# idiap/juicer

Measured on AMD Instinct MI355X. Metric: frames/sec decoded, higher is better.
Workload: dtype f32

## Files before the change

juicer_amd/build.py:

```python
from __future__ import annotations

import os
import shutil
import subprocess
import sys

HERE = os.path.dirname(os.path.abspath(__file__))
ROOT = os.path.dirname(HERE)
CSRC = os.path.join(HERE, "csrc")
LIB = os.path.join(HERE, "libjuicer_amd.so")
BATCH_TEST = os.path.join(HERE, "jd_batch_test")
BATCH_SRC = os.path.join(CSRC, "jd_batch_test.cpp")
SOURCES = [os.path.join(CSRC, "jd_host.cpp"), os.path.join(CSRC, "jd_device.hip"), os.path.join(CSRC, "jd_multi.cpp"),
           os.path.join(CSRC, "jd_compose.hip"), os.path.join(CSRC, "jd_broker.cpp")]
HEADERS_EXTRA = [os.path.join(CSRC, f) for f in ("jd_search.h", "jd_prep.h", "jd_lazy.h", "jd_labelsets.h", "jd_gmm.h", "jd_gc.h", "jd_resident.h", "jd_slot.h", "jd_host_resident.h", "jd_host_scoring.h", "jd_plan.h", "jd_host_launch.h", "jd_host_stream.h")]
HEADERS = [os.path.join(CSRC, "jd_internal.h"), os.path.join(ROOT, "include", "juicer_amd.h"),
           os.path.join(ROOT, "include", "juicer_amd_decoder.hpp"), BATCH_SRC]
FLAGS = ["--offload-arch=gfx950", "-O3", "-std=c++17", "-ffp-contract=off", "-fPIC", "-shared",
         "-Wall", "-Wno-unused-function"]


def hipcc() -> str:
    exe = shutil.which("hipcc") or "/opt/rocm/bin/hipcc"
    if not os.path.exists(exe):
        raise RuntimeError("hipcc not found: juicer_amd needs ROCm to build its HIP extension")
    return exe


def needs_build() -> bool:
    if not os.path.exists(LIB) or not os.path.exists(BATCH_TEST):
        return True
    t = os.path.getmtime(LIB)
    return any(os.path.getmtime(p) > t for p in SOURCES + HEADERS + HEADERS_EXTRA + [__file__])


def build(force: bool = False, verbose: bool = False) -> str:
    if not force and not needs_build():
        return LIB
    cmd = [hipcc()] + FLAGS + os.environ.get("JD_EXTRA_FLAGS", "").split() + ["-I", os.path.join(ROOT, "include"), "-I", CSRC, "-o", LIB] + SOURCES
    if verbose:
        print(" ".join(cmd), file=sys.stderr)
    subprocess.check_call(cmd)
    cmd2 = ["g++", "-O2", "-std=c++17", "-Wall", "-pthread", "-I", os.path.join(ROOT, "include"), "-o", BATCH_TEST, BATCH_SRC,
            "-L", HERE, "-ljuicer_amd", "-Wl,-rpath,$ORIGIN", "-Wl,-rpath-link," + "/opt/rocm/lib"]
    if verbose:
        print(" ".join(cmd2), file=sys.stderr)
    subprocess.check_call(cmd2)
    return LIB


if __name__ == "__main__":
    print(build(force="--force" in sys.argv, verbose=True))
```

juicer_amd/csrc/jd_gmm.h:

```cpp
#pragma once

#define JD_EXP2F_TAB                                                                              \
    0x3ff0000000000000ULL, 0x3fefd9b0d3158574ULL, 0x3fefb5586cf9890fULL, 0x3fef9301d0125b51ULL,   \
    0x3fef72b83c7d517bULL, 0x3fef54873168b9aaULL, 0x3fef387a6e756238ULL, 0x3fef1e9df51fdee1ULL,   \
    0x3fef06fe0a31b715ULL, 0x3feef1a7373aa9cbULL, 0x3feedea64c123422ULL, 0x3feece086061892dULL,   \
    0x3feebfdad5362a27ULL, 0x3feeb42b569d4f82ULL, 0x3feeab07dd485429ULL, 0x3feea47eb03a5585ULL,   \
    0x3feea09e667f3bcdULL, 0x3fee9f75e8ec5f74ULL, 0x3feea11473eb0187ULL, 0x3feea589994cce13ULL,   \
    0x3feeace5422aa0dbULL, 0x3feeb737b0cdc5e5ULL, 0x3feec49182a3f090ULL, 0x3feed503b23e255dULL,   \
    0x3feee89f995ad3adULL, 0x3feeff76f2fb5e47ULL, 0x3fef199bdd85529cULL, 0x3fef3720dcef9069ULL,   \
    0x3fef5818dcfba487ULL, 0x3fef7c97337b9b5fULL, 0x3fefa4afa2a490daULL, 0x3fefd0765b6e4540ULL
__device__ __constant__ unsigned long long jd_exp2f_tab[32] = {JD_EXP2F_TAB};
static const unsigned long long jd_exp2f_tab_host[32] = {JD_EXP2F_TAB};

__host__ __device__ __forceinline__ float jd_expf_impl(float x, const unsigned long long *tab)
{
    const double InvLn2N = 0x1.71547652b82fep+0 * 32.0;
    const double SHIFT = 0x1.8p+52;
    const double C0 = 0x1.c6af84b912394p-5 / 32.0 / 32.0 / 32.0;
    const double C1 = 0x1.ebfce50fac4f3p-3 / 32.0 / 32.0;
    const double C2 = 0x1.62e42ff0c52d6p-1 / 32.0;
    double z = InvLn2N * (double)x;
    double kd = z + SHIFT;
    unsigned long long ki;
    memcpy(&ki, &kd, sizeof ki);
    kd -= SHIFT;
    double r = z - kd;
    unsigned long long t = tab[ki & 31];
    t += ki << 47;
    double s;
    memcpy(&s, &t, sizeof s);
    double p = C0 * r + C1;
    double r2 = r * r;
    double y = C2 * r + 1.0;
    y = p * r2 + y;
    y = y * s;
    return (float)y;
}
__device__ __forceinline__ float jd_expf(float x) { return jd_expf_impl(x, jd_exp2f_tab); }

#define JD_LOG_TAB                                                                                          \
    0x3ff734f0c3e0de9fULL, 0xbfd7cc7f79e69000ULL, 0x3ff713786a2ce91fULL, 0xbfd76feec20d0000ULL,   \
    0x3ff6f26008fab5a0ULL, 0xbfd713e31351e000ULL, 0x3ff6d1a61f138c7dULL, 0xbfd6b85b38287800ULL,   \
    0x3ff6b1490bc5b4d1ULL, 0xbfd65d5590807800ULL, 0x3ff69147332f0cbaULL, 0xbfd602d076180000ULL,   \
    0x3ff6719f18224223ULL, 0xbfd5a8ca86909000ULL, 0x3ff6524f99a51ed9ULL, 0xbfd54f4356035000ULL,   \
    0x3ff63356aa8f24c4ULL, 0xbfd4f637c36b4000ULL, 0x3ff614b36b9ddc14ULL, 0xbfd49da7fda85000ULL,   \
    0x3ff5f66452c65c4cULL, 0xbfd445923989a800ULL, 0x3ff5d867b5912c4fULL, 0xbfd3edf439b0b800ULL,   \
    0x3ff5babccb5b90deULL, 0xbfd396ce448f7000ULL, 0x3ff59d61f2d91a78ULL, 0xbfd3401e17bda000ULL,   \
    0x3ff5805612465687ULL, 0xbfd2e9e2ef468000ULL, 0x3ff56397cee76bd3ULL, 0xbfd2941b3830e000ULL,   \
    0x3ff54725e2a77f93ULL, 0xbfd23ec58cda8800ULL, 0x3ff52aff42064583ULL, 0xbfd1e9e129279000ULL,   \
    0x3ff50f22dbb2bddfULL, 0xbfd1956d2b48f800ULL, 0x3ff4f38f4734ded7ULL, 0xbfd141679ab9f800ULL,   \
    0x3ff4d843cfde2840ULL, 0xbfd0edd094ef9800ULL, 0x3ff4bd3ec078a3c8ULL, 0xbfd09aa518db1000ULL,   \
    0x3ff4a27fc3e0258aULL, 0xbfd047e65263b800ULL, 0x3ff4880524d48434ULL, 0xbfcfeb224586f000ULL,   \
    0x3ff46dce1b192d0bULL, 0xbfcf474a7517b000ULL, 0x3ff453d9d3391854ULL, 0xbfcea4443d103000ULL,   \
    0x3ff43a2744b4845aULL, 0xbfce020d44e9b000ULL, 0x3ff420b54115f8fbULL, 0xbfcd60a22977f000ULL,   \
    0x3ff40782da3ef4b1ULL, 0xbfccc00104959000ULL, 0x3ff3ee8f5d57fe8fULL, 0xbfcc202956891000ULL,   \
    0x3ff3d5d9a00b4ce9ULL, 0xbfcb81178d811000ULL, 0x3ff3bd60c010c12bULL, 0xbfcae2c9ccd3d000ULL,   \
    0x3ff3a5242b75dab8ULL, 0xbfca45402e129000ULL, 0x3ff38d22cd9fd002ULL, 0xbfc9a877681df000ULL,   \
    0x3ff3755bc5847a1cULL, 0xbfc90c6d69483000ULL, 0x3ff35dce49ad36e2ULL, 0xbfc87120a645c000ULL,   \
    0x3ff34679984dd440ULL, 0xbfc7d68fb4143000ULL, 0x3ff32f5cceffcb24ULL, 0xbfc73cb83c627000ULL,   \
    0x3ff3187775a10d49ULL, 0xbfc6a39a9b376000ULL, 0x3ff301c8373e3990ULL, 0xbfc60b3154b7a000ULL,   \
    0x3ff2eb4ebb95f841ULL, 0xbfc5737d76243000ULL, 0x3ff2d50a0219a9d1ULL, 0xbfc4dc7b8fc23000ULL,   \
    0x3ff2bef9a8b7fd2aULL, 0xbfc4462c51d20000ULL, 0x3ff2a91c7a0c1babULL, 0xbfc3b08abc830000ULL,   \
    0x3ff293726014b530ULL, 0xbfc31b996b490000ULL, 0x3ff27dfa5757a1f5ULL, 0xbfc2875490a44000ULL,   \
    0x3ff268b39b1d3bbfULL, 0xbfc1f3b9f879a000ULL, 0x3ff2539d838ff5bdULL, 0xbfc160c8252ca000ULL,   \
    0x3ff23eb7aac9083bULL, 0xbfc0ce7f57f72000ULL, 0x3ff22a012ba940b6ULL, 0xbfc03cdc49fea000ULL,   \
    0x3ff2157996cc4132ULL, 0xbfbf57bdbc4b8000ULL, 0x3ff201201dd2fc9bULL, 0xbfbe370896404000ULL,   \
    0x3ff1ecf4494d480bULL, 0xbfbd17983ef94000ULL, 0x3ff1d8f5528f6569ULL, 0xbfbbf9674ed8a000ULL,   \
    0x3ff1c52311577e7cULL, 0xbfbadc79202f6000ULL, 0x3ff1b17c74cb26e9ULL, 0xbfb9c0c3e7288000ULL,   \
    0x3ff19e010c2c1ab6ULL, 0xbfb8a646b372c000ULL, 0x3ff18ab07bb670bdULL, 0xbfb78d01b3ac0000ULL,   \
    0x3ff1778a25efbcb6ULL, 0xbfb674f145380000ULL, 0x3ff1648d354c31daULL, 0xbfb55e0e6d878000ULL,   \
    0x3ff151b990275fddULL, 0xbfb4485cdea1e000ULL, 0x3ff13f0ea432d24cULL, 0xbfb333d94d6aa000ULL,   \
    0x3ff12c8b7210f9daULL, 0xbfb22079f8c56000ULL, 0x3ff11a3028ecb531ULL, 0xbfb10e4698622000ULL,   \
    0x3ff107fbda8434afULL, 0xbfaffa6c6ad20000ULL, 0x3ff0f5ee0f4e6bb3ULL, 0xbfadda8d4a774000ULL,   \
    0x3ff0e4065d2a9fceULL, 0xbfabbcece4850000ULL, 0x3ff0d244632ca521ULL, 0xbfa9a1894012c000ULL,   \
    0x3ff0c0a77ce2981aULL, 0xbfa788583302c000ULL, 0x3ff0af2f83c636d1ULL, 0xbfa5715e67d68000ULL,   \
    0x3ff09ddb98a01339ULL, 0xbfa35c8a49658000ULL, 0x3ff08cabaf52e7dfULL, 0xbfa149e364154000ULL,   \
    0x3ff07b9f2f4e28fbULL, 0xbf9e72c082eb8000ULL, 0x3ff06ab58c358f19ULL, 0xbf9a55f152528000ULL,   \
    0x3ff059eea5ecf92cULL, 0xbf963d62cf818000ULL, 0x3ff04949cdd12c90ULL, 0xbf9228fb8caa0000ULL,   \
    0x3ff038c6c6f0ada9ULL, 0xbf8c317b20f90000ULL, 0x3ff02865137932a9ULL, 0xbf8419355daa0000ULL,   \
    0x3ff0182427ea7348ULL, 0xbf781203c2ec0000ULL, 0x3ff008040614b195ULL, 0xbf60040979240000ULL,   \
    0x3fefe01ff726fa1aULL, 0x3f6feff384900000ULL, 0x3fefa11cc261ea74ULL, 0x3f87dc41353d0000ULL,   \
    0x3fef6310b081992eULL, 0x3f93cea3c4c28000ULL, 0x3fef25f63ceeadcdULL, 0x3f9b9fc114890000ULL,   \
    0x3feee9c8039113e7ULL, 0x3fa1b0d8ce110000ULL, 0x3feeae8078cbb1abULL, 0x3fa58a5bd001c000ULL,   \
    0x3fee741aa29d0c9bULL, 0x3fa95c8340d88000ULL, 0x3fee3a91830a99b5ULL, 0x3fad276aef578000ULL,   \
    0x3fee01e009609a56ULL, 0x3fb07598e598c000ULL, 0x3fedca01e577bb98ULL, 0x3fb253f5e30d2000ULL,   \
    0x3fed92f20b7c9103ULL, 0x3fb42edd8b380000ULL, 0x3fed5cac66fb5cceULL, 0x3fb606598757c000ULL,   \
    0x3fed272caa5ede9dULL, 0x3fb7da76356a0000ULL, 0x3fecf26e3e6b2ccdULL, 0x3fb9ab434e1c6000ULL,   \
    0x3fecbe6da2a77902ULL, 0x3fbb78c7bb0d6000ULL, 0x3fec8b266d37086dULL, 0x3fbd431332e72000ULL,   \
    0x3fec5894bd5d5804ULL, 0x3fbf0a3171de6000ULL, 0x3fec26b533bb9f8cULL, 0x3fc067152b914000ULL,   \
    0x3febf583eeece73fULL, 0x3fc147858292b000ULL, 0x3febc4fd75db96c1ULL, 0x3fc2266ecdca3000ULL,   \
    0x3feb951e0c864a28ULL, 0x3fc303d7a6c55000ULL, 0x3feb65e2c5ef3e2cULL, 0x3fc3dfc33c331000ULL,   \
    0x3feb374867c9888bULL, 0x3fc4ba366b7a8000ULL, 0x3feb094b211d304aULL, 0x3fc5933928d1f000ULL,   \
    0x3feadbe885f2ef7eULL, 0x3fc66acd2418f000ULL, 0x3feaaf1d31603da2ULL, 0x3fc740f8ec669000ULL,   \
    0x3fea82e63fd358a7ULL, 0x3fc815c0f51af000ULL, 0x3fea5740ef09738bULL, 0x3fc8e92954f68000ULL,   \
    0x3fea2c2a90ab4b27ULL, 0x3fc9bb3602f84000ULL, 0x3fea01a01393f2d1ULL, 0x3fca8bed1c2c0000ULL,   \
    0x3fe9d79f24db3c1bULL, 0x3fcb5b515c01d000ULL, 0x3fe9ae2505c7b190ULL, 0x3fcc2967ccbcc000ULL,   \
    0x3fe9852ef297ce2fULL, 0x3fccf635d5486000ULL, 0x3fe95cbaeea44b75ULL, 0x3fcdc1bd3446c000ULL,   \
    0x3fe934c69de74838ULL, 0x3fce8c01b8cfe000ULL, 0x3fe90d4f2f6752e6ULL, 0x3fcf5509c0179000ULL,   \
    0x3fe8e6528effd79dULL, 0x3fd00e6c121fb800ULL, 0x3fe8bfce9fcc007cULL, 0x3fd071b80e93d000ULL,   \
    0x3fe899c0dabec30eULL, 0x3fd0d46b9e867000ULL, 0x3fe87427aa2317fbULL, 0x3fd13687334bd000ULL,   \
    0x3fe84f00acb39a08ULL, 0x3fd1980d67234800ULL, 0x3fe82a49e8653e55ULL, 0x3fd1f8ffe0cc8000ULL,   \
    0x3fe8060195f40260ULL, 0x3fd2595fd7636800ULL, 0x3fe7e22563e0a329ULL, 0x3fd2b9300914a800ULL,   \
    0x3fe7beb377dcb5adULL, 0x3fd3187210436000ULL, 0x3fe79baa679725c2ULL, 0x3fd377266dec1800ULL,   \
    0x3fe77907f2170657ULL, 0x3fd3d54ffbaf3000ULL, 0x3fe756cadbd6130cULL, 0x3fd432eee32fe000ULL
__device__ __constant__ unsigned long long jd_log_tab[256] = {JD_LOG_TAB};
static const unsigned long long jd_log_tab_host[256] = {JD_LOG_TAB};

__host__ __device__ __forceinline__ double jd_u2d(unsigned long long u) { double d; memcpy(&d, &u, sizeof d); return d; }
__host__ __device__ __forceinline__ unsigned long long jd_d2u(double d) { unsigned long long u; memcpy(&u, &d, sizeof u); return u; }

__host__ __device__ inline double jd_log_libm_impl(double x, const unsigned long long *tab)
{
    const unsigned long long ix = jd_d2u(x);
    if (ix - 0x3fee000000000000ULL < 0x3ff1090000000000ULL - 0x3fee000000000000ULL) {
        if (ix == 0x3ff0000000000000ULL) return 0.0;
        const double r = x - 1.0, r2 = r * r, r3 = r * r2;
        double p = __builtin_fma(r, -0x1.ffffffffffdcbp-3, 0x1.5555555555577p-2);
        p = __builtin_fma(r2, 0x1.999999995dd0cp-3, p);
        double q = __builtin_fma(r, 0x1.24924a344de30p-3, -0x1.55555556745a7p-3);
        q = __builtin_fma(r2, -0x1.fffffa4423d65p-4, q);
        double s = __builtin_fma(r, -0x1.999eb43b068ffp-4, 0x1.c7184282ad6cap-4);
        s = __builtin_fma(r2, 0x1.78182f7afd085p-4, s);
        s = __builtin_fma(r3, -0x1.5521375d145cdp-4, s);
        s = __builtin_fma(s, r3, q);
        s = __builtin_fma(s, r3, p);
        const double rhi = __builtin_fma(-r, 0x1p27, __builtin_fma(r, 0x1p27, r));
        const double rlo = r - rhi;
        const double rr = rhi * rhi;
        const double hi = __builtin_fma(rr, -0.5, r);
        double lo = __builtin_fma(rr, -0.5, r - hi);
        lo = __builtin_fma(rlo * -0.5, r + rhi, lo);
        return hi + __builtin_fma(s, r3, lo);
    }
    const unsigned long long tmp = ix - 0x3fe6000000000000ULL;
    const int i = (int)((tmp >> 45) & 127);
    const double kd = (double)((long long)tmp >> 52);
    const double z = jd_u2d(ix - (tmp & (0xfffULL << 52)));
    const double invc = jd_u2d(tab[2 * i]), logc = jd_u2d(tab[2 * i + 1]);
    const double r = __builtin_fma(z, invc, -1.0);
    const double w = __builtin_fma(kd, 0x1.62e42fefa3800p-1, logc);
    const double hi = w + r;
    const double lo = __builtin_fma(kd, 0x1.ef35793c76730p-45, (w - hi) + r);
    const double r2 = r * r;
    const double p = __builtin_fma(__builtin_fma(r, -0x1.55575e506c89fp-3, 0x1.999b324f10111p-3), r2,
                                   __builtin_fma(r, -0x1.fffffffeb4590p-3, 0x1.555555551305bp-2));
    return __builtin_fma(r * r2, p, __builtin_fma(r2, -0x1.0000000000001p-1, lo)) + hi;
}

struct JdLogTab { double invc, logc; };
static inline void jd_fill_logtab(JdLogTab *t)
{
    for (int k = 0; k <= 128; ++k) {
        const double c = 1.0 + k / 128.0;
        t[k].invc = (k == 0) ? 1.0 : 1.0 / c;
        t[k].logc = (k == 0) ? 0.0 : (double)(-logl((long double)t[k].invc));
    }
}
__host__ __device__ __forceinline__ double jd_log1pe_table(double e, const JdLogTab *tab)
{
    const JdLogTab t = tab[(int)(e * 128.0 + 0.5)];
    const double r = __builtin_fma(1.0 + e, t.invc, -1.0);
    double q = 1.0 / 7.0;
    q = __builtin_fma(q, r, -1.0 / 6.0);
    q = __builtin_fma(q, r, 1.0 / 5.0);
    q = __builtin_fma(q, r, -1.0 / 4.0);
    q = __builtin_fma(q, r, 1.0 / 3.0);
    q = __builtin_fma(q, r, -1.0 / 2.0);
    q = __builtin_fma(q, r, 1.0);
    return t.logc + q * r;
}

__host__ __device__ __forceinline__ bool jd_log_add_gate(float a, float c, const JdLogTab *tab, const unsigned long long *etab,
                                                         float &x, float &d, double &y, float &n)
{
    const bool s = a < c;
    x = s ? c : a;
    d = (s ? a : c) - x;
    const double e = (double)jd_expf_impl(fmaxf(d, -19.0f), etab);
    y = 1.0 + e;
    const unsigned long long m = jd_d2u(jd_log1pe_table(e, tab));
    n = (float)((double)x + jd_u2d(m - 2));
    return d >= -18.42 && n != (float)((double)x + jd_u2d(m + 2));
}
__host__ __device__ __forceinline__ float jd_log_add_settle(float x, float d, float n)
{
    return d < -18.42 ? x : (d != d ? d : n);
}
__host__ __device__ __forceinline__ float jd_log_add_impl(float a, float c, const JdLogTab *tab, const unsigned long long *etab,
                                                          const unsigned long long *ltab)
{
    float x, d, n;
    double y;
    if (jd_log_add_gate(a, c, tab, etab, x, d, y, n)) n = (float)((double)x + jd_log_libm_impl(y, ltab));
    return jd_log_add_settle(x, d, n);
}
__device__ __forceinline__ float jd_log_add(float a, float c, const JdLogTab *tab)
{
    return jd_log_add_impl(a, c, tab, jd_exp2f_tab, jd_log_tab);
}


template <int DT>
__global__ __launch_bounds__(256) void jd_gmm_kernel(const float *__restrict__ feats,
                                                     const int *__restrict__ row_src, int n_rows,
                                                     const float *__restrict__ par,
                                                     const float *__restrict__ det,
                                                     const int *__restrict__ n_mix, int G, int M, int D,
                                                     float *__restrict__ ll, int skip_unused,
                                                     const JdLogTab *__restrict__ logtab)
{
    constexpr int DP = (DT > 0) ? (DT | 1) : 0;
    extern __shared__ __align__(16) char smem[];
    const int dp = (DT > 0) ? DP : (D | 1);
    float *sx = (float *)smem;
    float *so = sx + GMM_ROWS * dp;
    const int tid = threadIdx.x, lane = tid & 63;
    const int wid = __builtin_amdgcn_readfirstlane(tid >> 6);
    const int Dn = (DT > 0) ? DT : D;
    const int n_rt = (n_rows + GMM_ROWS - 1) / GMM_ROWS, n_gt = (G + GMM_GT - 1) / GMM_GT;
    for (int tile = blockIdx.x; tile < n_rt * n_gt; tile += gridDim.x) {
    const int gt = tile / n_rt;
    const int r0 = ((tile + gt) % n_rt) * GMM_ROWS;
    const int g0 = gt * GMM_GT;
    if (skip_unused && row_src[r0] < 0) continue;
    __syncthreads();

    for (int e = tid; e < GMM_ROWS * Dn; e += 256) {
        int r = e / Dn, j = e - r * Dn;
        int src = (r0 + r < n_rows) ? row_src[r0 + r] : -1;
        sx[r * dp + j] = (src >= 0) ? feats[(size_t)src * Dn + j] : 0.0f;
    }
    __syncthreads();

    float x[(DT > 0) ? DT : 1];
    if (DT > 0) {
#pragma unroll
        for (int j = 0; j < DT; ++j) x[j] = sx[lane * dp + j];
    }

    constexpr int GPW = GMM_GT / 4;
    for (int gi = 0; gi < GPW; ++gi) {
        const int gl = wid * GPW + gi;
        const int g = g0 + gl;
        float acc = LZ;
        if (g < G) {
            const int nm = n_mix[g];
            const float *pg = par + (size_t)g * M * Dn * 2;
            const float *dg = det + (size_t)g * M;
            for (int m = 0; m < nm; ++m) {
                const float *pm = pg + (size_t)m * Dn * 2;
                float sum = 0.0f;
                if (DT > 0) {
#pragma unroll
                    for (int j = 0; j < DT; ++j) {
                        float xmu = x[j] - pm[2 * j];
                        sum += xmu * xmu * pm[2 * j + 1];
                    }
                } else {
                    for (int j = 0; j < Dn; ++j) {
                        float xmu = sx[lane * dp + j] - pm[2 * j];
                        sum += xmu * xmu * pm[2 * j + 1];
                    }
                }
                float comp = (float)(-0.5 * (double)sum + (double)dg[m]);
                acc = jd_log_add(acc, comp, logtab);
            }
        }
        so[lane * (GMM_GT + 1) + gl] = acc;
    }
    __syncthreads();
    for (int e = tid; e < GMM_ROWS * GMM_GT; e += 256) {
        int r = e / GMM_GT, c = e - r * GMM_GT;
        if (r0 + r < n_rows && g0 + c < G) ll[(size_t)(r0 + r) * G + g0 + c] = so[r * (GMM_GT + 1) + c];
    }
    }
}


#define GMM_ROWS2 128
typedef float jd_f2 __attribute__((ext_vector_type(2)));
__host__ __device__ __forceinline__ void jd_log_add2x2(float &a0, float &a1, float c0, float c1, const JdLogTab *tab,
                                                       const unsigned long long *etab)
{
    float x0, x1, d0, d1, n0, n1;
    double y0, y1;
    const bool o0 = jd_log_add_gate(a0, c0, tab, etab, x0, d0, y0, n0);
    const bool o1 = jd_log_add_gate(a1, c1, tab, etab, x1, d1, y1, n1);
    a0 = o0 ? __builtin_nanf("") : jd_log_add_settle(x0, d0, n0);
    a1 = o1 ? __builtin_nanf("") : jd_log_add_settle(x1, d1, n1);
}

__device__ __noinline__ float jd_gmm_cell39(const float *__restrict__ feats, const int *__restrict__ row_src, int n_rows, int r,
                                            const float *__restrict__ pg, const float *__restrict__ dg, int nm,
                                            const JdLogTab *tab, const unsigned long long *etab)
{
    const int src = (r < n_rows) ? row_src[r] : -1;
    float acc = LZ;
    for (int m = 0; m < nm; ++m) {
        const float *pm = pg + (size_t)m * 39 * 2;
        float sum = 0.0f;
        for (int j = 0; j < 39; ++j) {
            const float u = ((src >= 0) ? feats[(size_t)src * 39 + j] : 0.0f) - pm[2 * j];
            const float z = u * u * pm[2 * j + 1];
            sum = (j == 0) ? z : sum + z;
        }
        const float c = (float)(-0.5 * (double)sum + (double)dg[m]);
        acc = (m == 0) ? (c <= LZ ? LZ : c) : jd_log_add_impl(acc, c, tab, etab, jd_log_tab);
    }
    return acc;
}

template <int GT>
__global__ __launch_bounds__(256, 4) void jd_gmm_kernel39(const float *__restrict__ feats,
                                                       const int *__restrict__ row_src, int n_rows,
                                                       const float *__restrict__ par,
                                                       const float *__restrict__ det,
                                                       const int *__restrict__ n_mix, int G, int M,
                                                       float *__restrict__ ll, int skip_unused,
                                                       const JdLogTab *__restrict__ logtab,
                                                       const int *__restrict__ rt_base, int n_rt_list)
{
    constexpr int DT = 39, DP = 39;
    extern __shared__ __align__(16) char smem[];
    JdLogTab *stab = (JdLogTab *)smem;
    unsigned long long *setab = (unsigned long long *)(smem + 130 * sizeof(JdLogTab));
    float *sx = (float *)(smem + 130 * sizeof(JdLogTab) + 32 * sizeof(unsigned long long));
    float *so = sx;
    const int tid = threadIdx.x, lane = tid & 63;
    const int wid = __builtin_amdgcn_readfirstlane(tid >> 6);
    for (int i = tid; i < 129; i += 256) stab[i] = logtab[i];
    if (tid < 32) setab[tid] = jd_exp2f_tab[tid];
    const int n_rt = rt_base ? n_rt_list : (n_rows + GMM_ROWS2 - 1) / GMM_ROWS2, n_gt = (G + GT - 1) / GT;
    for (int tile = blockIdx.x; tile < n_rt * n_gt; tile += gridDim.x) {
        const int gt = tile / n_rt;
        const int r0 = rt_base ? rt_base[(tile + gt) % n_rt] : ((tile + gt) % n_rt) * GMM_ROWS2;
        const int g0 = gt * GT;
        if (skip_unused && row_src[r0] < 0) continue;
        __syncthreads();
        for (int e = tid; e < GMM_ROWS2 * DT; e += 256) {
            const int r = e / DT, j = e - r * DT;
            const int src = (r0 + r < n_rows) ? row_src[r0 + r] : -1;
            sx[r * DP + j] = (src >= 0) ? feats[(size_t)src * DT + j] : 0.0f;
        }
        __syncthreads();
        jd_f2 x[DT];
#pragma unroll
        for (int j = 0; j < DT; ++j) { x[j].x = sx[lane * DP + j]; x[j].y = sx[(lane + 64) * DP + j]; }
        __syncthreads();
        constexpr int GPW = GT / 4;
        static_assert(GPW <= 16, "one bit per (state, frame) of a lane in open_cells");
        unsigned open_cells = 0;
        for (int gi = 0; gi < GPW; ++gi) {
            const int gl = wid * GPW + gi;
            const int g = g0 + gl;
            float acc0 = LZ, acc1 = LZ;
            if (g < G) {
                const int nm = n_mix[g];
                const float *pg = par + (size_t)g * M * DT * 2;
                const float *dg = det + (size_t)g * M;
                for (int m = 0; m < nm; ++m) {
                    const float *pm = pg + (size_t)m * DT * 2;
                    jd_f2 sum = {0.0f, 0.0f};
#pragma unroll
                    for (int j = 0; j < DT; j += 3) {
                        const jd_f2 mu0 = {pm[2 * j], pm[2 * j]}, iv0 = {pm[2 * j + 1], pm[2 * j + 1]};
                        const jd_f2 mu1 = {pm[2 * j + 2], pm[2 * j + 2]}, iv1 = {pm[2 * j + 3], pm[2 * j + 3]};
                        const jd_f2 mu2 = {pm[2 * j + 4], pm[2 * j + 4]}, iv2 = {pm[2 * j + 5], pm[2 * j + 5]};
                        const jd_f2 u0 = x[j] - mu0, u1 = x[j + 1] - mu1, u2 = x[j + 2] - mu2;
                        const jd_f2 w0 = u0 * u0, w1 = u1 * u1, w2 = u2 * u2;
                        const jd_f2 z0 = w0 * iv0, z1 = w1 * iv1, z2 = w2 * iv2;
                        if (j == 0) sum = z0; else sum += z0;
                        sum += z1; sum += z2;
                    }
                    const double dm = (double)dg[m];
                    const float c0 = (float)(-0.5 * (double)sum.x + dm), c1 = (float)(-0.5 * (double)sum.y + dm);
                    if (m == 0) { acc0 = c0 <= LZ ? LZ : c0; acc1 = c1 <= LZ ? LZ : c1; }
                    else jd_log_add2x2(acc0, acc1, c0, c1, stab, setab);
                }
            }
            so[lane * (GT + 1) + gl] = acc0;
            so[(lane + 64) * (GT + 1) + gl] = acc1;
            open_cells |= (acc0 != acc0 ? 1u << gi : 0u) | (acc1 != acc1 ? 1u << (16 + gi) : 0u);
        }
        for (unsigned o = open_cells; o; o &= o - 1) {
            const int b = __builtin_ctz(o), gl = wid * GPW + (b & 15), fr = b >> 4;
            const int g = g0 + gl;
            so[(lane + 64 * fr) * (GT + 1) + gl] = jd_gmm_cell39(feats, row_src, n_rows, r0 + lane + 64 * fr, par + (size_t)g * M * DT * 2,
                                                                det + (size_t)g * M, n_mix[g], stab, setab);
        }
        __syncthreads();
        for (int e = tid; e < GMM_ROWS2 * GT; e += 256) {
            const int r = e / GT, c = e - r * GT;
            if (r0 + r < n_rows && g0 + c < G) ll[(size_t)(r0 + r) * G + g0 + c] = so[r * (GT + 1) + c];
        }
    }
}


__device__ __forceinline__ float jd_log_add_fast(float a, float c)
{
    const float x = fmaxf(a, c), y = fminf(a, c);
    const float d = y - x;
    const float e = __builtin_amdgcn_exp2f(d * 1.44269504088896340736f);
    const float l = __builtin_amdgcn_logf(1.0f + e) * 0.69314718055994530942f;
    return d < -18.42f ? x : x + l;
}

template <int GT>
__global__ __launch_bounds__(256, 4) void jd_gmm_fast39(const float *__restrict__ feats, const int *__restrict__ row_src, int n_rows,
                                                      const float *__restrict__ par_fast, const float *__restrict__ det,
                                                      const int *__restrict__ n_mix, int G, int M, float *__restrict__ ll, int skip_unused,
                                                      const int *__restrict__ rt_base, int n_rt_list)
{
    constexpr int DT = 39, DP = 39;
    extern __shared__ __align__(16) char smem[];
    float *sx = (float *)smem;
    float *so = sx;
    const int tid = threadIdx.x, lane = tid & 63;
    const int wid = __builtin_amdgcn_readfirstlane(tid >> 6);
    const int n_rt = rt_base ? n_rt_list : (n_rows + GMM_ROWS2 - 1) / GMM_ROWS2, n_gt = (G + GT - 1) / GT;
    for (int tile = blockIdx.x; tile < n_rt * n_gt; tile += gridDim.x) {
        const int gt = tile / n_rt;
        const int r0 = rt_base ? rt_base[(tile + gt) % n_rt] : ((tile + gt) % n_rt) * GMM_ROWS2;
        const int g0 = gt * GT;
        if (skip_unused && row_src[r0] < 0) continue;
        __syncthreads();
        for (int e = tid; e < GMM_ROWS2 * DT; e += 256) {
            const int r = e / DT, j = e - r * DT;
            const int src = (r0 + r < n_rows) ? row_src[r0 + r] : -1;
            sx[r * DP + j] = (src >= 0) ? feats[(size_t)src * DT + j] : 0.0f;
        }
        __syncthreads();
        jd_f2 x[DT];
#pragma unroll
        for (int j = 0; j < DT; ++j) { x[j].x = sx[lane * DP + j]; x[j].y = sx[(lane + 64) * DP + j]; }
        __syncthreads();
        constexpr int GPW = GT / 4;
        for (int gi = 0; gi < GPW; ++gi) {
            const int gl = wid * GPW + gi;
            const int g = g0 + gl;
            float acc0 = LZ, acc1 = LZ;
            if (g < G) {
                const int nm = n_mix[g];
                const float *pg = par_fast + (size_t)g * M * DT * 2;
                const float *dg = det + (size_t)g * M;
                for (int m = 0; m < nm; ++m) {
                    const float *pm = pg + (size_t)m * DT * 2;
                    jd_f2 sum = {0.0f, 0.0f};
#pragma unroll
                    for (int j = 0; j < DT; ++j) {
                        const jd_f2 sj = {pm[2 * j], pm[2 * j]}, tj = {pm[2 * j + 1], pm[2 * j + 1]};
                        const jd_f2 u = __builtin_elementwise_fma(x[j], sj, tj);
                        sum = __builtin_elementwise_fma(u, u, sum);
                    }
                    const float dm = dg[m];
                    const float c0 = __builtin_fmaf(-0.5f, sum.x, dm), c1 = __builtin_fmaf(-0.5f, sum.y, dm);
                    if (m == 0) { acc0 = LZ < c0 ? c0 : LZ; acc1 = LZ < c1 ? c1 : LZ; }
                    else { acc0 = jd_log_add_fast(acc0, c0); acc1 = jd_log_add_fast(acc1, c1); }
                }
            }
            so[lane * (GT + 1) + gl] = acc0;
            so[(lane + 64) * (GT + 1) + gl] = acc1;
        }
        __syncthreads();
        for (int e = tid; e < GMM_ROWS2 * GT; e += 256) {
            const int r = e / GT, c = e - r * GT;
            if (r0 + r < n_rows && g0 + c < G) ll[(size_t)(r0 + r) * G + g0 + c] = so[r * (GT + 1) + c];
        }
    }
}


#define GMM_FAST_DC 8
#define GMM_FAST_DS 64
#define GMM_FAST_MB 8
template <int GT>
__global__ __launch_bounds__(256, 4) void jd_gmm_fast(const float *__restrict__ feats, const int *__restrict__ row_src, int n_rows,
                                                    const float *__restrict__ par_fast, const float *__restrict__ det,
                                                    const int *__restrict__ n_mix, int G, int M, int D, int DP, float *__restrict__ ll,
                                                    int skip_unused, const int *__restrict__ rt_base, int n_rt_list)
{
    constexpr int DC = GMM_FAST_DC, DS = GMM_FAST_DS, MB = GMM_FAST_MB, LS = DS + 1;
    extern __shared__ __align__(16) char smem[];
    float *sx = (float *)smem;
    const int tid = threadIdx.x, lane = tid & 63;
    const int wid = __builtin_amdgcn_readfirstlane(tid >> 6);
    const int n_slabs = (DP + DS - 1) / DS;
    const int n_rt = rt_base ? n_rt_list : (n_rows + GMM_ROWS2 - 1) / GMM_ROWS2, n_gt = (G + GT - 1) / GT;
    for (int tile = blockIdx.x; tile < n_rt * n_gt; tile += gridDim.x) {
        const int gt = tile / n_rt;
        const int r0 = rt_base ? rt_base[(tile + gt) % n_rt] : ((tile + gt) % n_rt) * GMM_ROWS2;
        const int g0 = gt * GT;
        if (skip_unused && row_src[r0] < 0) continue;
        auto stage = [&](int slab) {
            const int j0 = slab * DS, w = min(DS, DP - j0);
            __syncthreads();
            for (int e = tid; e < GMM_ROWS2 * w; e += 256) {
                const int r = e / w, k = e - r * w;
                const int src = (r0 + r < n_rows) ? row_src[r0 + r] : -1;
                sx[r * LS + k] = (src >= 0 && j0 + k < D) ? feats[(size_t)src * D + j0 + k] : 0.0f;
            }
            __syncthreads();
        };
        if (n_slabs == 1) stage(0);
        const float *x0 = sx + lane * LS, *x1 = sx + (lane + 64) * LS;
        constexpr int GPW = GT / 4;
        for (int gi = 0; gi < GPW; ++gi) {
            const int g = g0 + wid * GPW + gi;
            const int nm = (g < G) ? n_mix[g] : 0;
            const float *pg = par_fast + (size_t)(g < G ? g : 0) * M * DP * 2;
            const float *dg = det + (size_t)(g < G ? g : 0) * M;
            float acc0 = LZ, acc1 = LZ;
            const int m_end = (n_slabs == 1) ? nm : M;
            for (int m0 = 0; m0 < m_end; m0 += MB) {
                const int nb = min(MB, nm - m0);
                jd_f2 sum[MB];
#pragma unroll
                for (int mi = 0; mi < MB; ++mi) sum[mi] = jd_f2{0.0f, 0.0f};
                for (int slab = 0; slab < n_slabs; ++slab) {
                    if (n_slabs > 1) stage(slab);
                    if (nb <= 0) continue;
                    const int j0 = slab * DS, w = min(DS, DP - j0);
                    for (int jc = 0; jc < w; jc += DC) {
                        jd_f2 x[DC];
#pragma unroll
                        for (int k = 0; k < DC; ++k) { x[k].x = x0[jc + k]; x[k].y = x1[jc + k]; }
                        const float *pc = pg + ((size_t)m0 * DP + j0 + jc) * 2;
                        const unsigned ms = (unsigned)DP * 2u;
#pragma unroll
                        for (int mi = 0; mi < MB; ++mi) {
                            if (mi < nb) {
                                const float *pm = pc + (unsigned)mi * ms;
#pragma unroll
                                for (int k = 0; k < DC; ++k) {
                                    const jd_f2 sj = {pm[2 * k], pm[2 * k]}, tj = {pm[2 * k + 1], pm[2 * k + 1]};
                                    const jd_f2 u = __builtin_elementwise_fma(x[k], sj, tj);
                                    sum[mi] = __builtin_elementwise_fma(u, u, sum[mi]);
                                }
                            }
                        }
                    }
                }
#pragma unroll
                for (int mi = 0; mi < MB; ++mi) {
                    if (mi < nb) {
                        const float dm = dg[m0 + mi];
                        const float c0 = __builtin_fmaf(-0.5f, sum[mi].x, dm), c1 = __builtin_fmaf(-0.5f, sum[mi].y, dm);
                        if (m0 + mi == 0) { acc0 = LZ < c0 ? c0 : LZ; acc1 = LZ < c1 ? c1 : LZ; }
                        else { acc0 = jd_log_add_fast(acc0, c0); acc1 = jd_log_add_fast(acc1, c1); }
                    }
                }
            }
            if (g < G) {
                if (r0 + lane < n_rows) ll[(size_t)(r0 + lane) * G + g] = acc0;
                if (r0 + lane + 64 < n_rows) ll[(size_t)(r0 + lane + 64) * G + g] = acc1;
            }
        }
    }
}
```

Measured before the change: 2.586 million.

## Software-pipeline GMM mixture parameter loads across head, mid and tail chunks

New measurement: 2.533 million. 0.98x the previous value.

```diff
diff --git a/juicer_amd/build.py b/juicer_amd/build.py
--- a/juicer_amd/build.py
+++ b/juicer_amd/build.py
@@ -13,7 +13,7 @@
 BATCH_SRC = os.path.join(CSRC, "jd_batch_test.cpp")
 SOURCES = [os.path.join(CSRC, "jd_host.cpp"), os.path.join(CSRC, "jd_device.hip"), os.path.join(CSRC, "jd_multi.cpp"),
            os.path.join(CSRC, "jd_compose.hip"), os.path.join(CSRC, "jd_broker.cpp")]
-HEADERS_EXTRA = [os.path.join(CSRC, f) for f in ("jd_search.h", "jd_prep.h", "jd_lazy.h", "jd_labelsets.h", "jd_gmm.h", "jd_gc.h", "jd_resident.h", "jd_slot.h", "jd_host_resident.h", "jd_host_scoring.h", "jd_plan.h", "jd_host_launch.h", "jd_host_stream.h")]
+HEADERS_EXTRA = [os.path.join(CSRC, f) for f in ("jd_search.h", "jd_prep.h", "jd_lazy.h", "jd_labelsets.h", "jd_gmm.h", "jd_gmm_next.h", "jd_gc.h", "jd_resident.h", "jd_slot.h", "jd_host_resident.h", "jd_host_scoring.h", "jd_plan.h", "jd_host_launch.h", "jd_host_stream.h")]
 HEADERS = [os.path.join(CSRC, "jd_internal.h"), os.path.join(ROOT, "include", "juicer_amd.h"),
            os.path.join(ROOT, "include", "juicer_amd_decoder.hpp"), BATCH_SRC]
 FLAGS = ["--offload-arch=gfx950", "-O3", "-std=c++17", "-ffp-contract=off", "-fPIC", "-shared",
diff --git a/juicer_amd/csrc/jd_gmm.h b/juicer_amd/csrc/jd_gmm.h
--- a/juicer_amd/csrc/jd_gmm.h
+++ b/juicer_amd/csrc/jd_gmm.h
@@ -1,4 +1,6 @@
 #pragma once
+
+#include "jd_gmm_next.h"
 
 #define JD_EXP2F_TAB                                                                              \
     0x3ff0000000000000ULL, 0x3fefd9b0d3158574ULL, 0x3fefb5586cf9890fULL, 0x3fef9301d0125b51ULL,   \
@@ -278,6 +280,15 @@
 
 
 #define GMM_ROWS2 128
+#ifndef JD_GMM_HEAD
+#define JD_GMM_HEAD 18
+#endif
+#ifndef JD_GMM_MID
+#define JD_GMM_MID 30
+#endif
+#ifndef JD_GMM_TOUCH
+#define JD_GMM_TOUCH ((77 - JD_GMM_HEAD) / 16 + 2)
+#endif
 typedef float jd_f2 __attribute__((ext_vector_type(2)));
 __host__ __device__ __forceinline__ void jd_log_add2x2(float &a0, float &a1, float c0, float c1, const JdLogTab *tab,
                                                        const unsigned long long *etab)
@@ -350,29 +361,76 @@
         constexpr int GPW = GT / 4;
         static_assert(GPW <= 16, "one bit per (state, frame) of a lane in open_cells");
         unsigned open_cells = 0;
+#define JD_GMM_AFTER(off, v) asm volatile("" : "+s"(off) : "v"(v))
+        constexpr int H = JD_GMM_HEAD, MID = JD_GMM_MID, T = DT * 2 - H - MID;
+        static_assert(H % 6 == 0 && MID % 6 == 0 && T >= 12, "whole groups of three dimensions; the tail has two");
+        float head[H];
+        {
+            const JdMix first = jd_gmm_first_mix(g0, GPW, wid, 0, n_mix, G, M);
+            const float *pf = par + (first.g >= 0 ? ((size_t)first.g * M + first.m) * (DT * 2) : 0);
+#pragma unroll
+            for (int i = 0; i < H; ++i) head[i] = first.g >= 0 ? pf[i] : 0.0f;
+        }
         for (int gi = 0; gi < GPW; ++gi) {
             const int gl = wid * GPW + gi;
             const int g = g0 + gl;
             float acc0 = LZ, acc1 = LZ;
             if (g < G) {
                 const int nm = n_mix[g];
-                const float *pg = par + (size_t)g * M * DT * 2;
                 const float *dg = det + (size_t)g * M;
+                const JdMix after = jd_gmm_first_mix(g0, GPW, wid, gi + 1, n_mix, G, M);
+                const size_t o_g = (size_t)g * M * (DT * 2);
+                const size_t o_after = after.g >= 0 ? ((size_t)after.g * M + after.m) * (DT * 2) : o_g + (size_t)(nm - 1) * (DT * 2);
                 for (int m = 0; m < nm; ++m) {
-                    const float *pm = pg + (size_t)m * DT * 2;
+                    const size_t o_m = o_g + (size_t)m * (DT * 2);
+                    const float *pm = par + o_m;
+                    const float *pn = par + (jd_gmm_step_mix(g, m, nm, M, after).g == g ? o_m + DT * 2 : o_after);
                     jd_f2 sum = {0.0f, 0.0f};
-#pragma unroll
-                    for (int j = 0; j < DT; j += 3) {
-                        const jd_f2 mu0 = {pm[2 * j], pm[2 * j]}, iv0 = {pm[2 * j + 1], pm[2 * j + 1]};
-                        const jd_f2 mu1 = {pm[2 * j + 2], pm[2 * j + 2]}, iv1 = {pm[2 * j + 3], pm[2 * j + 3]};
-                        const jd_f2 mu2 = {pm[2 * j + 4], pm[2 * j + 4]}, iv2 = {pm[2 * j + 5], pm[2 * j + 5]};
+                    auto group = [&](int j, const float *p) {
+                        const jd_f2 mu0 = {p[0], p[0]}, iv0 = {p[1], p[1]};
+                        const jd_f2 mu1 = {p[2], p[2]}, iv1 = {p[3], p[3]};
+                        const jd_f2 mu2 = {p[4], p[4]}, iv2 = {p[5], p[5]};
                         const jd_f2 u0 = x[j] - mu0, u1 = x[j + 1] - mu1, u2 = x[j + 2] - mu2;
                         const jd_f2 w0 = u0 * u0, w1 = u1 * u1, w2 = u2 * u2;
                         const jd_f2 z0 = w0 * iv0, z1 = w1 * iv1, z2 = w2 * iv2;
                         if (j == 0) sum = z0; else sum += z0;
                         sum += z1; sum += z2;
-                    }
-                    const double dm = (double)dg[m];
+                    };
+                    float mid[MID], tail[T];
+#pragma unroll
+                    for (int i = 0; i < MID; ++i) mid[i] = pm[H + i];
+#if JD_GMM_TOUCH
+                    unsigned long long touch[JD_GMM_TOUCH];
+#pragma unroll
+                    for (int i = 0; i < JD_GMM_TOUCH; ++i) __builtin_memcpy(&touch[i], pn + (H + i * 16 < DT * 2 - 2 ? H + i * 16 : DT * 2 - 2), 8);
+#endif
+                    __builtin_amdgcn_sched_barrier(0);
+#pragma unroll
+                    for (int j = 0; j < H / 2; j += 3) group(j, head + 2 * j);
+                    __builtin_amdgcn_sched_barrier(0);
+                    group(H / 2, mid);
+                    size_t o_tail = 0;
+                    JD_GMM_AFTER(o_tail, sum.x);
+#if JD_GMM_TOUCH
+#pragma unroll
+                    for (int i = 0; i < JD_GMM_TOUCH; ++i) asm volatile("" ::"s"(touch[i]));
+#endif
+#pragma unroll
+                    for (int i = 0; i < T; ++i) tail[i] = (pm + o_tail)[H + MID + i];
+                    const float dgm = (dg + o_tail)[m];
+                    __builtin_amdgcn_sched_barrier(0);
+#pragma unroll
+                    for (int j = H / 2 + 3; j < (H + MID) / 2; j += 3) group(j, mid + 2 * j - H);
+                    __builtin_amdgcn_sched_barrier(0);
+                    group((H + MID) / 2, tail);
+                    size_t o_head = 0;
+                    JD_GMM_AFTER(o_head, sum.x);
+#pragma unroll
+                    for (int i = 0; i < H; ++i) head[i] = (pn + o_head)[i];
+                    __builtin_amdgcn_sched_barrier(0);
+#pragma unroll
+                    for (int j = (H + MID) / 2 + 3; j < DT; j += 3) group(j, tail + 2 * j - H - MID);
+                    const double dm = (double)dgm;
                     const float c0 = (float)(-0.5 * (double)sum.x + dm), c1 = (float)(-0.5 * (double)sum.y + dm);
                     if (m == 0) { acc0 = c0 <= LZ ? LZ : c0; acc1 = c1 <= LZ ? LZ : c1; }
                     else jd_log_add2x2(acc0, acc1, c0, c1, stab, setab);
diff --git a/juicer_amd/csrc/jd_gmm_next.h b/juicer_amd/csrc/jd_gmm_next.h
--- /dev/null
+++ b/juicer_amd/csrc/jd_gmm_next.h
@@ -0,0 +1,28 @@
+#pragma once
+
+#ifdef __HIPCC__
+#define JD_NEXT_HD __host__ __device__ __forceinline__
+#else
+#define JD_NEXT_HD inline
+#endif
+
+struct JdMix { int g, m; };
+
+JD_NEXT_HD JdMix jd_gmm_first_mix(int g0, int GPW, int wid, int gi, const int *n_mix, int G, int M)
+{
+    for (; gi < GPW; ++gi) {
+        const int g = g0 + wid * GPW + gi;
+        if (g >= G) break;
+        if (n_mix[g] > 0 && M > 0) return JdMix{g, 0};
+    }
+    return JdMix{-1, 0};
+}
+JD_NEXT_HD JdMix jd_gmm_step_mix(int g, int m, int nm, int M, JdMix after)
+{
+    return (m + 1 < nm && m + 1 < M) ? JdMix{g, m + 1} : after;
+}
+JD_NEXT_HD JdMix jd_gmm_next_mix(int g0, int GPW, int wid, int gi, int m, const int *n_mix, int G, int M)
+{
+    const int g = g0 + wid * GPW + gi;
+    return jd_gmm_step_mix(g, m, n_mix[g], M, jd_gmm_first_mix(g0, GPW, wid, gi + 1, n_mix, G, M));
+}
```
